# xxxupeng/stereo_toolbox

Measured on AMD Instinct MI355X. Metric: stereo pairs/sec @ 540x960 D=192 (GwcNet_GC fwd+bwd), higher is better.
Workload: dtype f32; 1 GPU; GwcNet_GC(maxdisp=192) train step: fwd+bwd+allreduce+Adam, 576x960 pairs (reference pad_to_2x shape), batch 1/GPU, fp32, synthetic randn inputs, deterministic filler weights; global_batch=1, parallelism=dp1, grad_sync=none (single rank: flat fp32 buffer packed, no collective), launch=eager, optimizer=torch.optim.Adam(fused=True)

## Files before the change

### include/stx_hip.h

```cpp
#ifndef STX_HIP_H
#define STX_HIP_H
#ifdef __cplusplus
extern "C" {
#endif

const char* stx_last_error(void);
const char* stx_build_info(void);
int stx_get_tuning(const char* name);
int stx_set_tuning(const char* name, int value);

int stx_cost_volume_fwd(const float* Lg, const float* Rg, int Cg, int G, const float* Lc, const float* Rc, int Cc,
                        const float* scale, float* vol, int B, int H, int W, int D, int mask_left, void* stream);
int stx_group_normalize_fwd(const float* x, float* y, int B, int C, int G, int HW, float out_scale, void* stream);
int stx_group_normalize_bwd(const float* x, const float* gy, float* gx, int B, int C, int G, int HW, float out_scale, void* stream);
int stx_cost_volume_bwd(const float* gvol, const float* Lg, const float* Rg, int Cg, int G, int Cc, float* gLg,
                        float* gRg, float* gLc, float* gRc, int B, int H, int W, int D, int mask_left, void* stream);

int stx_head_fwd(const float* cost, float* disp, float* stats, int B, int Dc, int Hc, int Wc, int D, int H, int W,
                 void* stream);
long long stx_head_bwd_workspace_floats(int B, int Dc, int H, int W);
int stx_head_bwd(const float* gdisp, const float* cost, const float* disp, const float* stats, float* gcost,
                 float* workspace, int B, int Dc, int Hc, int Wc, int D, int H, int W, void* stream);
int stx_head_fwd2(const float* cost, float* disp, float* stats, int B, int Dc, int Hc, int Wc, int D, int H, int W,
                  int align_corners, void* stream);
// ... 71 lines not shown
                    float* running_mean, float* running_var, float momentum, float eps, float* scale, float* shift,
                    float* mean, float* invstd, void* stream);
int stx_bn_finalize_groups(const float* partials, int nrows, int C, double count, const float* gamma, const float* beta,
                           float* running_mean, float* running_var, float momentum, float eps, float* out, int groups,
                           void* stream);
int stx_bn_apply(const float* z1, const float* scale1, const float* shift1, const float* z2, const float* scale2,
                 const float* shift2, float* out, long long nvox, int C, int relu, int groups, void* stream);
int stx_bn_bwd_reduce(const float* gy, const float* y, const float* z1, const float* mean1, const float* invstd1,
                      const float* z2, const float* mean2, const float* invstd2, float* partials, float* sums,
                      long long nvox, int C, int relu, void* stream);
int stx_bn_bwd_apply(const float* gy, const float* y, const float* z1, const float* mean1, const float* invstd1,
                     const float* gamma1, const float* z2, const float* mean2, const float* invstd2,
                     const float* gamma2, const float* sums, float* dz1, float* dz2, float* gout, long long nvox, int C,
                     int relu, void* stream);
int stx_bn_bwd_reduce2(const float* gy, const float* y, const float* z1, const float* mean1, const float* invstd1,
                       const float* z2, const float* mean2, const float* invstd2, const float* scale1,
                       const float* shift1, const float* scale2, const float* shift2, float* partials, float* sums,
                       long long nvox, int C, int relu, int groups, void* stream);
int stx_bn_bwd_apply2(const float* gy, const float* y, const float* z1, const float* mean1, const float* invstd1,
                      const float* gamma1, const float* z2, const float* mean2, const float* invstd2,
                      const float* gamma2, const float* scale1, const float* shift1, const float* scale2,
                      const float* shift2, const float* sums, float* dz1, float* dz2, float* gout, long long nvox,
                      int C, int relu, int groups, void* stream);

int stx_pad_normalize_u8(const unsigned char* img, float* out, int B, int H, int W, int Hp, int Wp, int top,
                         const float* mean3, const float* std3, void* stream);

int stx_sampled_volume_fwd(const float* Lg, const float* Rg, int Cg, int G, const float* Lc, const float* Rc, int Cc,
                           const float* samples, float* vol, int B, int H, int W, int S, int CTp, void* stream);
int stx_sampled_volume_bwd(const float* gvol, const float* Lg, const float* Rg, int Cg, int G, int Cc,
                           const float* samples, float* gLg, float* gRg, float* gLc, float* gRc, int B, int H, int W,
                           int S, int CTp, void* stream);

int stx_warp_fwd(const float* x, const float* disp, float* out, int B, int C, int H, int W, void* stream);
int stx_warp_bwd(const float* gout, const float* x, const float* disp, float* gx, float* gdisp, int B, int C, int H, int W,
                 void* stream);
int stx_corr_volume_fwd(const float* ref, const float* tgt, float* vol, int B, int C, int H, int W, int maxdisp, int groups,
                        void* stream);
int stx_corr_volume_bwd(const float* gvol, const float* ref, const float* tgt, float* gref, float* gtgt, int B, int C, int H,
                        int W, int maxdisp, int groups, void* stream);
int stx_disparity_variance_fwd(const float* x, const float* disp, const float* samples, float* out, int B, int D, int HW,
                               void* stream);
int stx_disparity_variance_bwd(const float* g, const float* x, const float* disp, const float* samples, float* gx, float* gdisp,
                               float* gsamples, int B, int D, int HW, void* stream);

long long stx_geo_pyramid_floats(long long rows, int len, int C, int levels);
// ... 19 lines not shown
```

### stereo_toolbox_amd/_capi.py

```python
import ctypes
import os
import threading

import torch

_P = ctypes.c_void_p
_I = ctypes.c_int
_F = ctypes.c_float
_L = ctypes.c_longlong

SIGNATURES = {
    "stx_get_tuning": [ctypes.c_char_p],
    "stx_set_tuning": [ctypes.c_char_p, _I],
    "stx_cost_volume_fwd": [_P, _P, _I, _I, _P, _P, _I, _P, _P, _I, _I, _I, _I, _I, _P],
    "stx_cost_volume_bwd": [_P, _P, _P, _I, _I, _I, _P, _P, _P, _P, _I, _I, _I, _I, _I, _P],
    "stx_group_normalize_fwd": [_P, _P, _I, _I, _I, _I, _F, _P],
    "stx_group_normalize_bwd": [_P, _P, _P, _I, _I, _I, _I, _F, _P],
    "stx_head_fwd": [_P, _P, _P, _I, _I, _I, _I, _I, _I, _I, _P],
    "stx_head_bwd_workspace_floats": [_I, _I, _I, _I],
    "stx_head_bwd": [_P, _P, _P, _P, _P, _P, _I, _I, _I, _I, _I, _I, _I, _P],
    "stx_head_fwd2": [_P, _P, _P, _I, _I, _I, _I, _I, _I, _I, _I, _P],
    "stx_head_bwd2": [_P, _P, _P, _P, _P, _P, _I, _I, _I, _I, _I, _I, _I, _I, _P],
    "stx_softargmax_fwd": [_P, _P, _I, _I, _I, _P],
    "stx_argmax_fwd": [_P, _P, _I, _I, _I, _P],
# ... 43 lines not shown
    "stx_disparity_variance_fwd": [_P, _P, _P, _P, _I, _I, _I, _P],
    "stx_disparity_variance_bwd": [_P, _P, _P, _P, _P, _P, _P, _I, _I, _I, _P],
    "stx_sampled_volume_fwd": [_P, _P, _I, _I, _P, _P, _I, _P, _P, _I, _I, _I, _I, _I, _P],
    "stx_sampled_volume_bwd": [_P, _P, _P, _I, _I, _I, _P, _P, _P, _P, _P, _I, _I, _I, _I, _I, _P],
    "stx_geo_pyramid_floats": [_L, _I, _I, _I],
    "stx_geo_corr_fwd": [_P, _P, _P, _I, _I, _I, _I, _I, _I, _P],
    "stx_geo_corr_bwd": [_P, _P, _P, _P, _P, _I, _I, _I, _I, _I, _I, _P],
    "stx_geo_pyramid_fwd": [_P, _P, _I, _I, _I, _I, _I, _I, _P],
    "stx_geo_pyramid_bwd": [_P, _P, _I, _I, _I, _I, _I, _I, _P],
    "stx_geo_lookup_fwd": [_P, _P, _P, _P, _P, _I, _I, _I, _I, _I, _I, _I, _I, _P],
    "stx_geo_lookup_bwd": [_P, _P, _P, _P, _P, _I, _I, _I, _I, _I, _I, _I, _I, _P],
    "stx_context_upsample_fwd": [_P, _P, _P, _I, _I, _I, _P],
    "stx_context_upsample_bwd": [_P, _P, _P, _P, _P, _I, _I, _I, _P],
    "stx_bn_reduce_blocks": [],
    "stx_bn_stats_rows": [_L, _I],
    "stx_bn_stats": [_P, _P, _L, _I, _I, _P],
    "stx_bn_finalize": [_P, _I, _I, ctypes.c_double, _P, _P, _P, _P, _F, _F, _P, _P, _P, _P, _P],
    "stx_bn_finalize_groups": [_P, _I, _I, ctypes.c_double, _P, _P, _P, _P, _F, _F, _P, _I, _P],
    "stx_bn_apply": [_P, _P, _P, _P, _P, _P, _P, _L, _I, _I, _I, _P],
    "stx_bn_bwd_reduce": [_P, _P, _P, _P, _P, _P, _P, _P, _P, _P, _L, _I, _I, _P],
    "stx_bn_bwd_apply": [_P, _P, _P, _P, _P, _P, _P, _P, _P, _P, _P, _P, _P, _P, _L, _I, _I, _P],
    "stx_bn_bwd_reduce2": [_P] * 14 + [_L, _I, _I, _I, _P],
    "stx_bn_bwd_apply2": [_P] * 18 + [_L, _I, _I, _I, _P],
}
_RET_CHARP = ("stx_last_error", "stx_build_info")


class StxError(RuntimeError):
    pass


class StxLib:

    def __init__(self, path):
        if not os.path.exists(path):
            raise StxError(
                f"HIP library not found: {path}. Build it with `python -m stereo_toolbox_amd.build` "
                "(hipcc, gfx950). There is no CPU fallback for the cost-volume hot path.")
        self.path = path
        self._dll = ctypes.CDLL(path)
        for name in _RET_CHARP:
            fn = getattr(self._dll, name)
            fn.restype = ctypes.c_char_p
            fn.argtypes = []
        self._fns = {}
        for name, argtypes in SIGNATURES.items():
# ... 47 lines not shown
```

### stereo_toolbox_amd/csrc/bn.hip

```cpp
#include "stx_common.h"
#include <stdlib.h>

namespace {

constexpr int BN_THREADS = 256;
constexpr int BN_RED_BLOCKS = 1024;

__device__ __forceinline__ double bn_block_sum(double v, double* red, int tid) {
    red[tid] = v;
    __syncthreads();
    for (int s = BN_THREADS / 2; s > 0; s >>= 1) {
        if (tid < s) red[tid] += red[tid + s];
        __syncthreads();
    }
    const double r = red[0];
    __syncthreads();
    return r;
}

__global__ __launch_bounds__(BN_THREADS) void bn_finalize_kernel(
    const float* __restrict__ partials, int nrows, int C, double count, const float* __restrict__ gamma,
    const float* __restrict__ beta, float* __restrict__ running_mean, float* __restrict__ running_var,
    float momentum, float eps, float* __restrict__ scale, float* __restrict__ shift, float* __restrict__ mean_out,
    float* __restrict__ invstd_out, int groups) {
    __shared__ double red[BN_THREADS];
    const int c = blockIdx.x, tid = threadIdx.x;
    for (int g = 0; g < groups; ++g, partials += (size_t)nrows * 2 * C, scale += C, shift += C, mean_out += C, invstd_out += C) {
    double s1 = 0.0, s2 = 0.0;
    for (int r = tid; r < nrows; r += BN_THREADS) {
        s1 += (double)partials[(size_t)r * 2 * C + c];
        s2 += (double)partials[(size_t)r * 2 * C + C + c];
    }
    s1 = bn_block_sum(s1, red, tid);
    s2 = bn_block_sum(s2, red, tid);
    if (tid == 0) {
        const double mean = s1 / count;
        double var = s2 / count - mean * mean;
        if (var < 0.0) var = 0.0;
        const float invstd = (float)(1.0 / sqrt(var + (double)eps));
        const float g = gamma ? gamma[c] : 1.f, bt = beta ? beta[c] : 0.f;
        const float sc = g * invstd;
        scale[c] = sc;
        shift[c] = bt - (float)mean * sc;
        mean_out[c] = (float)mean;
        invstd_out[c] = invstd;
        if (running_mean) running_mean[c] = (1.f - momentum) * running_mean[c] + momentum * (float)mean;
        if (running_var) {
            const double unb = count > 1.0 ? var * count / (count - 1.0) : var;
            running_var[c] = (1.f - momentum) * running_var[c] + momentum * (float)unb;
        }
    }
    }
}

constexpr int BN_FIN_THREADS = 512;

__device__ __forceinline__ double bn_shfl_down_f64(double v, int delta) {
    union { double d; float f[2]; } a, b;
    a.d = v;
    b.f[0] = __shfl_down(a.f[0], delta);
    b.f[1] = __shfl_down(a.f[1], delta);
    return b.d;
}

__global__ __launch_bounds__(BN_FIN_THREADS) void bn_finalize4_kernel(
    const float* __restrict__ partials, int nrows, int C, double count, const float* __restrict__ gamma,
    const float* __restrict__ beta, float* __restrict__ running_mean, float* __restrict__ running_var,
    float momentum, float eps, float* __restrict__ scale, float* __restrict__ shift, float* __restrict__ mean_out,
    float* __restrict__ invstd_out, int groups) {
    __shared__ double red[BN_FIN_THREADS / 64][8];
    const int c0 = blockIdx.x * 4, tid = threadIdx.x, lane = tid & 63, wave = tid >> 6;
    for (int g = 0; g < groups; ++g, partials += (size_t)nrows * 2 * C, scale += C, shift += C, mean_out += C, invstd_out += C) {
    if (g) __syncthreads();
    double acc[8] = {0.0, 0.0, 0.0, 0.0, 0.0, 0.0, 0.0, 0.0};
    const float* p = partials + c0;
#pragma unroll 4
    for (int r = tid; r < nrows; r += BN_FIN_THREADS) {
        const float4 a = stx_ld4(p + (size_t)r * 2 * C), b = stx_ld4(p + (size_t)r * 2 * C + C);
        acc[0] += (double)a.x; acc[1] += (double)a.y; acc[2] += (double)a.z; acc[3] += (double)a.w;
        acc[4] += (double)b.x; acc[5] += (double)b.y; acc[6] += (double)b.z; acc[7] += (double)b.w;
    }
#pragma unroll
    for (int k = 0; k < 8; ++k) {
#pragma unroll
        for (int d = 32; d > 0; d >>= 1) acc[k] += bn_shfl_down_f64(acc[k], d);
        if (lane == 0) red[wave][k] = acc[k];
    }
    __syncthreads();
    if (tid < 4) {
        double s1 = 0.0, s2 = 0.0;
        for (int w = 0; w < BN_FIN_THREADS / 64; ++w) { s1 += red[w][tid]; s2 += red[w][4 + tid]; }
        const int c = c0 + tid;
        const double mean = s1 / count;
        double var = s2 / count - mean * mean;
        if (var < 0.0) var = 0.0;
        const float invstd = (float)(1.0 / sqrt(var + (double)eps));
        const float g = gamma ? gamma[c] : 1.f, bt = beta ? beta[c] : 0.f;
        const float sc = g * invstd;
        scale[c] = sc;
        shift[c] = bt - (float)mean * sc;
        mean_out[c] = (float)mean;
        invstd_out[c] = invstd;
        if (running_mean) running_mean[c] = (1.f - momentum) * running_mean[c] + momentum * (float)mean;
        if (running_var) {
            const double unb = count > 1.0 ? var * count / (count - 1.0) : var;
            running_var[c] = (1.f - momentum) * running_var[c] + momentum * (float)unb;
        }
    }
    }
}

__global__ __launch_bounds__(BN_THREADS) void bn_apply_kernel(
    const float* __restrict__ z1, const float* __restrict__ scale1, const float* __restrict__ shift1,
    const float* __restrict__ z2, const float* __restrict__ scale2, const float* __restrict__ shift2,
    float* __restrict__ out, size_t nquads, int CQ, int relu) {
    {
        const size_t go = (size_t)blockIdx.y * nquads * 4, gc = (size_t)blockIdx.y * CQ * 4;
        z1 += go; out += go; scale1 += gc; shift1 += gc;
        if (z2) z2 += go;
        if (scale2) { scale2 += gc; shift2 += gc; }
    }
    for (size_t i = (size_t)blockIdx.x * BN_THREADS + threadIdx.x; i < nquads; i += (size_t)gridDim.x * BN_THREADS) {
        const int cq = (int)(i % CQ) * 4;
        float4 v = stx_ld4(z1 + i * 4);
        const float4 a = stx_ld4(scale1 + cq), b = stx_ld4(shift1 + cq);
        v.x = fmaf(v.x, a.x, b.x); v.y = fmaf(v.y, a.y, b.y); v.z = fmaf(v.z, a.z, b.z); v.w = fmaf(v.w, a.w, b.w);
        if (z2) {
            float4 u = stx_ld4(z2 + i * 4);
            if (scale2) {
                const float4 a2 = stx_ld4(scale2 + cq), b2 = stx_ld4(shift2 + cq);
                u.x = fmaf(u.x, a2.x, b2.x); u.y = fmaf(u.y, a2.y, b2.y);
                u.z = fmaf(u.z, a2.z, b2.z); u.w = fmaf(u.w, a2.w, b2.w);
            }
            v.x += u.x; v.y += u.y; v.z += u.z; v.w += u.w;
        }
        if (relu) {
            v.x = stx_act(v.x, relu); v.y = stx_act(v.y, relu); v.z = stx_act(v.z, relu); v.w = stx_act(v.w, relu);
        }
        stx_st4(out + i * 4, v);
    }
}

__global__ __launch_bounds__(BN_THREADS) void bn_bwd_reduce_kernel(
    const float* __restrict__ gy, const float* __restrict__ y, const float* __restrict__ z1,
    const float* __restrict__ mean1, const float* __restrict__ invstd1, const float* __restrict__ z2,
    const float* __restrict__ mean2, const float* __restrict__ invstd2, const float* __restrict__ sc1,
    const float* __restrict__ sh1, const float* __restrict__ sc2, const float* __restrict__ sh2, float* __restrict__ partials,
    size_t nvox, int C, int relu) {
    __shared__ float red[BN_THREADS * 12];
    const int tid = threadIdx.x;
    const int CQ = C >> 2;
    const int cq = tid % CQ, vl = tid / CQ, VPB = BN_THREADS / CQ;
    {
        const size_t go = (size_t)blockIdx.y * nvox * C, gc = (size_t)blockIdx.y * C;
        gy += go; z1 += go; mean1 += gc; invstd1 += gc;
        if (y) y += go;
        if (z2) z2 += go;
        if (mean2) { mean2 += gc; invstd2 += gc; }
        if (sc1) { sc1 += gc; sh1 += gc; }
        if (sc2) { sc2 += gc; sh2 += gc; }
        partials += (size_t)blockIdx.y * gridDim.x * 3 * C;
    }
    const float4 m1 = stx_ld4(mean1 + 4 * cq), i1 = stx_ld4(invstd1 + 4 * cq);
    float4 m2 = make_float4(0.f, 0.f, 0.f, 0.f), i2 = m2;
    const bool has2 = z2 && mean2;
    if (has2) { m2 = stx_ld4(mean2 + 4 * cq); i2 = stx_ld4(invstd2 + 4 * cq); }
    const bool remask = relu && !y;
    float4 a1 = m2, b1 = m2, a2 = m2, b2 = m2;
    if (remask) {
        a1 = stx_ld4(sc1 + 4 * cq); b1 = stx_ld4(sh1 + 4 * cq);
        if (has2) { a2 = stx_ld4(sc2 + 4 * cq); b2 = stx_ld4(sh2 + 4 * cq); }
    }
// ... 17 lines not shown
            } else {
                yy = stx_ld4(y + o);
            }
            g.x = stx_act_bwd(g.x, yy.x, relu); g.y = stx_act_bwd(g.y, yy.y, relu);
            g.z = stx_act_bwd(g.z, yy.z, relu); g.w = stx_act_bwd(g.w, yy.w, relu);
        }
        s[0] += g.x; s[1] += g.y; s[2] += g.z; s[3] += g.w;
        s[4] = fmaf(g.x, (a.x - m1.x) * i1.x, s[4]); s[5] = fmaf(g.y, (a.y - m1.y) * i1.y, s[5]);
        s[6] = fmaf(g.z, (a.z - m1.z) * i1.z, s[6]); s[7] = fmaf(g.w, (a.w - m1.w) * i1.w, s[7]);
        if (has2) {
            s[8] = fmaf(g.x, (c.x - m2.x) * i2.x, s[8]); s[9] = fmaf(g.y, (c.y - m2.y) * i2.y, s[9]);
            s[10] = fmaf(g.z, (c.z - m2.z) * i2.z, s[10]); s[11] = fmaf(g.w, (c.w - m2.w) * i2.w, s[11]);
        }
    }
#pragma unroll
    for (int k = 0; k < 12; ++k) red[k * BN_THREADS + tid] = s[k];
    __syncthreads();
    for (int idx = tid; idx < 12 * CQ; idx += BN_THREADS) {
        const int k = idx / CQ, q = idx % CQ;
        float t = 0.f;
        for (int j = q; j < BN_THREADS; j += CQ) t += red[k * BN_THREADS + j];
        partials[((size_t)blockIdx.x * 3 + (k >> 2)) * C + 4 * q + (k & 3)] = t;
    }
}

__global__ __launch_bounds__(BN_THREADS) void bn_stats_kernel(const float* __restrict__ z, float* __restrict__ partials,
                                                              size_t nvox, int C) {
    __shared__ float red[BN_THREADS * 8];
    const int tid = threadIdx.x;
    const int CQ = C >> 2;
    const int cq = tid % CQ, vl = tid / CQ, VPB = BN_THREADS / CQ;
    z += (size_t)blockIdx.y * nvox * C;
    partials += (size_t)blockIdx.y * gridDim.x * 2 * C;
    float s[8];
#pragma unroll
    for (int k = 0; k < 8; ++k) s[k] = 0.f;
    const size_t step = (size_t)gridDim.x * VPB;
    size_t v = vl < VPB ? (size_t)blockIdx.x * VPB + vl : nvox;
    for (; v + 3 * step < nvox; v += 4 * step) {
        float4 a[4];
#pragma unroll
        for (int u = 0; u < 4; ++u) a[u] = stx_ld4(z + (v + u * step) * C + 4 * cq);
#pragma unroll
        for (int u = 0; u < 4; ++u) {
            s[0] += a[u].x; s[1] += a[u].y; s[2] += a[u].z; s[3] += a[u].w;
            s[4] = fmaf(a[u].x, a[u].x, s[4]); s[5] = fmaf(a[u].y, a[u].y, s[5]);
            s[6] = fmaf(a[u].z, a[u].z, s[6]); s[7] = fmaf(a[u].w, a[u].w, s[7]);
        }
    }
    for (; v < nvox; v += step) {
        const float4 a = stx_ld4(z + v * C + 4 * cq);
        s[0] += a.x; s[1] += a.y; s[2] += a.z; s[3] += a.w;
        s[4] = fmaf(a.x, a.x, s[4]); s[5] = fmaf(a.y, a.y, s[5]); s[6] = fmaf(a.z, a.z, s[6]); s[7] = fmaf(a.w, a.w, s[7]);
    }
#pragma unroll
    for (int k = 0; k < 8; ++k) red[k * BN_THREADS + tid] = s[k];
    __syncthreads();
    for (int idx = tid; idx < 8 * CQ; idx += BN_THREADS) {
        const int k = idx / CQ, q = idx % CQ;
        float t = 0.f;
        for (int j = q; j < BN_THREADS; j += CQ) t += red[k * BN_THREADS + j];
        partials[((size_t)blockIdx.x * 2 + (k >> 2)) * C + 4 * q + (k & 3)] = t;
    }
}

__global__ __launch_bounds__(BN_THREADS) void bn_colsum_kernel(const float* __restrict__ partials, int nrows, int M,
                                                               float* __restrict__ sums, int groups) {
    __shared__ double red[BN_THREADS];
    const int m = blockIdx.x, tid = threadIdx.x;
    float tot = 0.f;
    for (int g = 0; g < groups; ++g) {
        const float* p = partials + (size_t)g * nrows * M;
        double s = 0.0;
        for (int r = tid; r < nrows; r += BN_THREADS) s += (double)p[(size_t)r * M + m];
        s = bn_block_sum(s, red, tid);
        if (tid == 0) {
            sums[(size_t)g * M + m] = (float)s;
            tot += (float)s;
        }
    }
    if (groups > 1 && tid == 0) sums[(size_t)groups * M + m] = tot;
}

__global__ __launch_bounds__(BN_THREADS) void bn_bwd_apply_kernel(
    const float* __restrict__ gy, const float* __restrict__ y, const float* __restrict__ z1,
    const float* __restrict__ mean1, const float* __restrict__ invstd1, const float* __restrict__ gamma1,
// ... 98 lines not shown
extern "C" int stx_bn_finalize_groups(const float* partials, int nrows, int C, double count, const float* gamma,
                                      const float* beta, float* running_mean, float* running_var, float momentum, float eps,
                                      float* out, int groups, void* stream) {
    stx_begin();
    STX_REQUIRE(partials && nrows > 0 && C > 0 && count > 0 && out && groups >= 1, "bn_finalize_groups: bad args");
    const size_t gc = (size_t)groups * C;
    return bn_finalize_launch(partials, nrows, C, count, gamma, beta, running_mean, running_var, momentum, eps, out, out + gc,
                              out + 2 * gc, out + 3 * gc, groups, stream);
}

extern "C" int stx_bn_stats_rows(long long nvox, int C) {
    stx_begin();
    if (C < 4 || C % 4 != 0 || C / 4 > BN_THREADS || nvox < 1) return 0;
    const long long vpb = BN_THREADS / (C / 4);
    const long long g = (nvox + 4 * vpb - 1) / (4 * vpb);
    return (int)(g > 256 ? 256 : (g < 1 ? 1 : g));
}

extern "C" int stx_bn_stats(const float* z, float* partials, long long nvox, int C, int groups, void* stream) {
    stx_begin();
    STX_REQUIRE(z && partials && nvox > 0 && groups >= 1 && groups <= 65535, "bn_stats: bad args");
    STX_REQUIRE(C >= 4 && C % 4 == 0 && C / 4 <= BN_THREADS, "bn_stats: C=%d unsupported (a multiple of 4, at most 1024)", C);
    hipLaunchKernelGGL(bn_stats_kernel, dim3(stx_bn_stats_rows(nvox, C), groups), dim3(BN_THREADS), 0, (hipStream_t)stream, z,
                       partials, (size_t)nvox, C);
    return stx_check_launch("bn_stats");
}

extern "C" int stx_bn_apply(const float* z1, const float* scale1, const float* shift1, const float* z2,
                            const float* scale2, const float* shift2, float* out, long long nvox, int C, int relu,
                            int groups, void* stream) {
    stx_begin();
    STX_REQUIRE(z1 && scale1 && shift1 && out && nvox > 0 && C > 0 && C % 4 == 0, "bn_apply: bad args (C=%d)", C);
    STX_REQUIRE(!scale2 || (z2 && shift2), "bn_apply: second affine needs z2 and shift2");
    STX_REQUIRE(groups >= 1 && groups <= 65535, "bn_apply: groups=%d", groups);
    const size_t nquads = (size_t)nvox * (C / 4);
    hipLaunchKernelGGL(bn_apply_kernel, dim3(bn_grid(nquads), groups), dim3(BN_THREADS), 0, (hipStream_t)stream, z1, scale1,
                       shift1, z2, scale2, shift2, out, nquads, C / 4, relu);
    return stx_check_launch("bn_apply");
}

extern "C" int stx_bn_bwd_reduce2(const float* gy, const float* y, const float* z1, const float* mean1,
                                  const float* invstd1, const float* z2, const float* mean2, const float* invstd2,
                                  const float* scale1, const float* shift1, const float* scale2, const float* shift2,
                                  float* partials, float* sums, long long nvox, int C, int relu, int groups, void* stream) {
    stx_begin();
    STX_REQUIRE(gy && z1 && mean1 && invstd1 && partials && sums && nvox > 0, "bn_bwd_reduce: null operand");
    STX_REQUIRE(groups >= 1 && groups <= 65535, "bn_bwd_reduce: groups=%d", groups);
    STX_REQUIRE(C >= 4 && C % 4 == 0 && C / 4 <= BN_THREADS, "bn_bwd_reduce: C=%d unsupported (a multiple of 4, at most 1024)", C);
    STX_REQUIRE(!relu || y || (scale1 && shift1 && (!(z2 && mean2) || (scale2 && shift2))),
                "bn_bwd_reduce: the relu mask needs y or the forward pass's scale / shift vectors");
    STX_REQUIRE(relu != 2 || !y, "bn_bwd_reduce: Mish (activation code 2) differentiates the pre-activation value: pass y = NULL and the scale / shift vectors");
    hipStream_t st = (hipStream_t)stream;
    const int nblk = ((long long)nvox * C <= (9ll << 19)) ? BN_RED_BLOCKS / 4 : BN_RED_BLOCKS;
    hipLaunchKernelGGL(bn_bwd_reduce_kernel, dim3(nblk, groups), dim3(BN_THREADS), 0, st, gy, y, z1, mean1, invstd1,
                       z2, mean2, invstd2, scale1, shift1, scale2, shift2, partials, (size_t)nvox, C, relu);
    int rc = stx_check_launch("bn_bwd_reduce");
    if (rc) return rc;
    hipLaunchKernelGGL(bn_colsum_kernel, dim3(3 * C), dim3(BN_THREADS), 0, st, partials, nblk, 3 * C, sums, groups);
    return stx_check_launch("bn_colsum");
}

extern "C" int stx_bn_bwd_apply2(const float* gy, const float* y, const float* z1, const float* mean1,
                                 const float* invstd1, const float* gamma1, const float* z2, const float* mean2,
                                 const float* invstd2, const float* gamma2, const float* scale1, const float* shift1,
                                 const float* scale2, const float* shift2, const float* sums, float* dz1, float* dz2,
                                 float* gout, long long nvox, int C, int relu, int groups, void* stream) {
    stx_begin();
    STX_REQUIRE(gy && z1 && mean1 && invstd1 && sums && dz1 && nvox > 0 && C % 4 == 0, "bn_bwd_apply: bad args");
    STX_REQUIRE(groups >= 1 && groups <= 65535, "bn_bwd_apply: groups=%d", groups);
    STX_REQUIRE(!relu || y || (scale1 && shift1 && (!(z2 && mean2 && dz2) || (scale2 && shift2))),
                "bn_bwd_apply: the relu mask needs y or the forward pass's scale / shift vectors");
    STX_REQUIRE(relu != 2 || !y, "bn_bwd_apply: Mish (activation code 2) differentiates the pre-activation value: pass y = NULL and the scale / shift vectors");
    const size_t nquads = (size_t)nvox * (C / 4);
    hipLaunchKernelGGL(bn_bwd_apply_kernel, dim3(bn_grid(nquads), groups), dim3(BN_THREADS), 0, (hipStream_t)stream, gy, y, z1,
                       mean1, invstd1, gamma1, z2, mean2, invstd2, gamma2, scale1, shift1, scale2, shift2, sums, dz1, dz2,
                       gout, nquads, C, relu, (float)(1.0 / (double)nvox));
    return stx_check_launch("bn_bwd_apply");
}

extern "C" int stx_bn_bwd_reduce(const float* gy, const float* y, const float* z1, const float* mean1,
                                 const float* invstd1, const float* z2, const float* mean2, const float* invstd2,
                                 float* partials, float* sums, long long nvox, int C, int relu, void* stream) {
// ... 12 lines not shown
```

### stereo_toolbox_amd/csrc/stx_runtime.hip

```cpp
#include "stx_common.h"
#include <stdarg.h>
#include <stdio.h>

static thread_local char g_err[512] = "";

int stx_set_error(int code, const char* fmt, ...) {
    va_list ap;
    va_start(ap, fmt);
    vsnprintf(g_err, sizeof(g_err), fmt, ap);
    va_end(ap);
    return code;
}

int stx_check_launch(const char* what) {
    hipError_t e = hipGetLastError();
    if (e != hipSuccess) return stx_set_error(STX_ERR_LAUNCH, "%s: launch failed: %s", what, hipGetErrorString(e));
    return STX_OK;
}

extern "C" const char* stx_last_error(void) { return g_err; }

extern "C" const char* stx_build_info(void) {
#ifdef STX_HIPEMU
    return "stx-hipemu (host SIMT emulator build: tests only)";
// ... 12 lines not shown
    {"STX_SV_BWD_V1", 0}, {"STX_DWCONV_ROLL", 1},
};
struct TuneInit {
    TuneInit() {
        for (int i = 0; i < STX_TUNE_COUNT; ++i)
            if (const char* e = getenv(g_tune[i].name)) g_tune[i].value = atoi(e);
    }
} g_tune_init;
}

int stx_tune(StxTune id) { return g_tune[id].value; }

extern "C" int stx_get_tuning(const char* name) {
    for (int i = 0; i < STX_TUNE_COUNT; ++i)
        if (name && !strcmp(name, g_tune[i].name)) return g_tune[i].value;
    return -1;
}

extern "C" int stx_set_tuning(const char* name, int value) {
    for (int i = 0; i < STX_TUNE_COUNT; ++i)
        if (name && !strcmp(name, g_tune[i].name)) { g_tune[i].value = value; return STX_OK; }
    return stx_set_error(STX_ERR_ARG, "stx_set_tuning: unknown switch %s", name ? name : "(null)");
}
```

### stereo_toolbox_amd/models/features2d.py

```python
import math
import os
import threading

import torch
import torch.nn as nn
import torch.nn.functional as F

from .. import ops
from ..aggregation import _bn_state, _fold


def channels_last_weights_(module):
    for m in module.modules():
        if isinstance(m, nn.Conv2d) and m.weight.dim() == 4:
            m.weight.data = m.weight.data.contiguous(memory_format=torch.channels_last)
    return module


def fused_glue(x, *bns):
    if os.environ.get("STX_FEAT2D_FUSED", "1") == "0":
        return False
    if x.dtype != torch.float32 or not ops.on_device(x):
        return False
    if ops.autocast_active():
# ... 22 lines not shown

    def __exit__(self, *exc):
        view_groups._tls.n = self.old
        return False


def _nhwc(t):
    v = t.permute(0, 2, 3, 1)
    return v if v.is_contiguous() else v.contiguous()


def cat_features(parts):
    parts = list(parts)
    if (os.environ.get("STX_FEAT2D_FUSED", "1") != "0" and os.environ.get("STX_FEAT2D_FUSED_CAT", "1") != "0" and 2 <= len(parts) <= 4
            and all(p.dtype == torch.float32 and ops.on_device(p) and p.shape[1] % 4 == 0
                    and p.is_contiguous(memory_format=torch.channels_last) for p in parts)):
        return ops.cat_channels([_nhwc(p) for p in parts]).permute(0, 3, 1, 2)
    return torch.cat(parts, dim=1)


def own_conv2d(x, conv):
    return (os.environ.get("STX_FEAT2D_CONV", "1") != "0" and x.dtype == torch.float32 and ops.on_device(x)
            and ops.conv2d_supported(conv) and x.shape[0] % view_groups.current() == 0)


def conv_bn_act(x, conv, bn, relu=False, residual=None, second=None):
    G = view_groups.current()
    part = None
    if bn.training and own_conv2d(x, conv):
        zl, part = ops.Conv2dFn.apply(x, conv.weight, G)
        z = zl.permute(0, 3, 1, 2)
    else:
        z = F.conv2d(x, conv.weight, conv.bias, conv.stride, conv.padding, conv.dilation, conv.groups)
        zl = _nhwc(z)
    if not bn.training:
        if torch.is_grad_enabled() and (z.requires_grad or bn.weight.requires_grad):
            raise ops.StxError("conv_bn_act: eval-mode BatchNorm under autograd has no fused backward -- gate the call "
                               "with fused_glue() over every BatchNorm of the block")
        sc, sh = _fold(bn)
        if second is not None:
            sc2, sh2 = _fold(second[1])
            y = ops.bn_apply(zl, sc, sh, _nhwc(second[0]), sc2, sh2, relu)
        else:
            y = ops.bn_apply(zl, sc, sh, None if residual is None else _nhwc(residual), None, None, relu)
        return y.permute(0, 3, 1, 2)
    st = _bn_state(bn, part if part is not None else ops.bn_stats(zl.detach(), G), zl.numel() // zl.shape[-1] // G, steps=G)
    if second is not None:
        z2l = _nhwc(second[0])
        bn2 = second[1]
        st2 = _bn_state(bn2, ops.bn_stats(z2l.detach(), G), z2l.numel() // z2l.shape[-1] // G, steps=G)
        y = ops.BnActFn.apply(zl, bn.weight, bn.bias, z2l, bn2.weight, bn2.bias, None, relu, st, st2, G)
    else:
        y = ops.BnActFn.apply(zl, bn.weight, bn.bias, None, None, None, None if residual is None else _nhwc(residual),
                              relu, st, None, G)
    return y.permute(0, 3, 1, 2)


def convbn_relu_chain(seq, x):
    i, n = 0, len(seq)
    while i < n:
        m = seq[i]
        if isinstance(m, nn.Sequential) and len(m) == 2 and isinstance(m[0], nn.Conv2d):
            relu = i + 1 < n and isinstance(seq[i + 1], nn.ReLU)
            x = conv_bn_act(x, m[0], m[1], relu=relu)
            i += 2 if relu else 1
        else:
            x = m(x)
            i += 1
    return x


def _chain_bns(seq):
    return [m[1] for m in seq if isinstance(m, nn.Sequential) and len(m) == 2 and isinstance(m[0], nn.Conv2d)]
# ... 130 lines not shown
```

### stereo_toolbox_amd/ops.py

```python
import ctypes

import torch

from ._capi import StxError, get_lib

_P = ctypes.c_void_p


class _DevPtr(ctypes.c_void_p):
    """A device pointer that remembers the device of the tensor it came from: _call() reads the launch device off its
    own arguments, so nothing survives between launches (an exception between building the arguments and the launch
    cannot leak state into the next one)."""


def _stream(dev=None):
    return _P(torch.cuda.current_stream(dev).cuda_stream)


def _p(t):
    if t is None:
        return None
    p = _DevPtr(t.data_ptr())
    p.dev = t.device
    return p
# ... 693 lines not shown
def bn_finalize(partials, count, gamma, beta, running_mean, running_var, momentum, eps, groups=1):
    C = partials.shape[-1]
    out = torch.empty(4, groups, C, dtype=torch.float32, device=partials.device)
    _call("stx_bn_finalize_groups", _p(partials), partials.shape[-3], C, float(count), _p(gamma), _p(beta),
          _p(running_mean), _p(running_var), float(momentum), float(eps), _p(out), groups)
    return list(out.unbind(0)) if groups > 1 else list(out[:, 0].unbind(0))


@fp32_region
def bn_stats(z, groups=1):
    _chk(z, "z")
    C = z.shape[-1]
    nvox = z.numel() // C // groups
    if groups < 1 or z.shape[0] % groups:
        raise StxError(f"bn_stats: leading axis {z.shape[0]} does not split into {groups} groups")
    rows = get_lib().raw("stx_bn_stats_rows")(nvox, C)
    if rows <= 0:
        raise StxError(f"bn_stats: C={C} unsupported")
    part = torch.empty(groups, rows, 2, C, dtype=torch.float32, device=z.device)
    _call("stx_bn_stats", _p(z), _p(part), nvox, C, groups)
    return part if groups > 1 else part[0]


def _sync_bn_partials(partials, count, group, world):
    import torch.distributed as dist
    tot = partials.double().sum(0)
    dist.all_reduce(tot, group=group)
    hi = tot.float()
    lo = (tot - hi.double()).float()
    return torch.stack((hi, lo)).contiguous(), count * world


@fp32_region
def bn_apply(z1, scale1, shift1, z2=None, scale2=None, shift2=None, relu=False, groups=1):
    out = torch.empty_like(z1)
    C = z1.shape[-1]
    _call("stx_bn_apply", _p(z1), _p(scale1), _p(shift1), _p(z2), _p(scale2), _p(shift2), _p(out),
          z1.numel() // C // groups, C, int(relu), groups)
    return out


class BnActFn(torch.autograd.Function):

    @staticmethod
    def forward(ctx, z1, gamma1, beta1, z2, gamma2, beta2, residual, relu, bn1, bn2, groups=1, defer=False):
        G = int(groups)
        ctx.defer = bool(defer)

        def affine(gamma, beta, bn):
            if bn["training"]:
                partials, count = bn["partials"], bn["count"]
                if bn.get("sync"):
                    if G > 1:
                        raise StxError("BnActFn: SyncBatchNorm with groups is not wired (SyncBN runs the views separately)")
                    partials, count = _sync_bn_partials(partials, count, *bn["sync"])
                return bn_finalize(partials, count, gamma, beta, bn["running_mean"], bn["running_var"], bn["momentum"],
                                   bn["eps"], G)
            invstd = torch.rsqrt(bn["running_var"] + bn["eps"])
            scale = gamma * invstd
            res = (scale, beta - bn["running_mean"] * scale, bn["running_mean"].clone(), invstd)
            return res if G == 1 else [t.unsqueeze(0).expand(G, -1).contiguous() for t in res]

        relu = int(relu)
        if relu == 2 and residual is not None:
            raise StxError("BnActFn: Mish with a plain residual is not wired (no model of the family uses it)")
        if G < 1 or z1.shape[0] % G:
            raise StxError(f"BnActFn: leading axis {z1.shape[0]} does not split into {G} groups")
        sc1, sh1, m1, i1 = affine(gamma1, beta1, bn1)
        two = z2 is not None
        if two:
            sc2, sh2, m2, i2 = affine(gamma2, beta2, bn2)
            y = bn_apply(z1, sc1, sh1, z2, sc2, sh2, relu, G)
        else:
# ... 2 lines not shown
        ctx.relu, ctx.two, ctx.has_res, ctx.groups = relu, two, residual is not None, G
        ctx.train1 = bn1["training"]
        ctx.train2 = bn2["training"] if two else False
        ctx.sync = bn1.get("sync") or (bn2.get("sync") if two else None)
        ctx.remask = bool(relu) and residual is None
        keep_y = y if (relu and not ctx.remask) else None
        ctx.save_for_backward(z1, gamma1, m1, i1, z2, gamma2, m2, i2, keep_y, sc1 if ctx.remask else None,
                              sh1 if ctx.remask else None, sc2 if (ctx.remask and two) else None,
                              sh2 if (ctx.remask and two) else None)
        return y

    @staticmethod
    def backward(ctx, gy):
        z1, gamma1, m1, i1, z2, gamma2, m2, i2, y, sc1, sh1, sc2, sh2 = ctx.saved_tensors
        gy = gy.contiguous()
        G = ctx.groups
        C = z1.shape[-1]
        nvox = z1.numel() // C // G
        lib = get_lib()
        NB = lib.raw("stx_bn_reduce_blocks")()
        part = _WS.get("bnred", G * NB * 3 * C, z1.device)
        sums_all = torch.empty(G + (1 if G > 1 else 0), 3, C, dtype=torch.float32, device=z1.device)
        sums = sums_all[:G]
        _call("stx_bn_bwd_reduce2", _p(gy), _p(y), _p(z1), _p(m1), _p(i1), _p(z2) if ctx.two else None,
              _p(m2) if ctx.two else None, _p(i2) if ctx.two else None, _p(sc1), _p(sh1), _p(sc2), _p(sh2), _p(part),
              _p(sums_all), nvox, C, int(ctx.relu), G)
        if not ctx.needs_input_grad[0] and not ctx.two and not ctx.has_res:
            tot = sums_all[G] if G > 1 else sums_all[0]
            return (None, tot[1], tot[0], None, None, None, None, None, None, None, None, None)
        if (ctx.defer and not ctx.two and not ctx.has_res and ctx.relu in (0, 1) and ctx.train1 and not ctx.sync and G == 1
                and (not ctx.relu or ctx.remask)):
            alias = gy.view_as(gy)
            pend = _PendingBn()
            pend.g, pend.z, pend.scale, pend.shift, pend.mean, pend.invstd = alias, z1, sc1, sh1, m1, i1
            pend.gamma, pend.sums, pend.inv_n, pend.act = gamma1, sums, 1.0 / nvox, int(ctx.relu)
            if pend.scale is None:
                pend.scale = pend.shift = m1
            _defer_pending_bn(alias, pend)
            tot = sums_all[0]
            return (alias, tot[1], tot[0], None, None, None, None, None, None, None, None, None)
        dz1 = torch.empty_like(z1)
        dz2 = torch.empty_like(z2) if ctx.two else None
        gres = torch.empty_like(z1) if (ctx.has_res and ctx.relu) else None
        use = sums
        if ctx.sync:
            import torch.distributed as dist
            use = sums.clone()
# ... 735 lines not shown
```

Before: 0.1786 pairs/s.

## Fuse BN partial-sum reduction and finalize into the stats kernels via last-block counters

Adds a last-block-done reduction scheme. Per-block partial rows are reduced in double into a pooled scratch slot guarded by atomic counters, and the final block either finalizes the BN affine parameters (forward stats) or writes the column sums (backward reduce). This removes the separate colsum and finalize kernel launches for each 2D-feature BN layer in both forward and backward. In exchange it adds a ring of 16 reusable counter/scratch slots, which could collide if more than 16 reductions are in flight, and it adds extra serial work in the last block.

```diff
diff --git a/include/stx_hip.h b/include/stx_hip.h
--- a/include/stx_hip.h
+++ b/include/stx_hip.h
@@ -117,6 +117,14 @@
                       const float* gamma2, const float* scale1, const float* shift1, const float* scale2,
                       const float* shift2, const float* sums, float* dz1, float* dz2, float* gout, long long nvox,
                       int C, int relu, int groups, void* stream);
+int stx_bn_bwd_reduce_sums(const float* gy, const float* y, const float* z1, const float* mean1, const float* invstd1,
+                           const float* z2, const float* mean2, const float* invstd2, const float* scale1,
+                           const float* shift1, const float* scale2, const float* shift2, float* partials, float* sums,
+                           long long nvox, int C, int relu, int groups, void* stream);
+int stx_bn_stats_finalize(const float* z, float* partials, long long nvox, int C, int groups, double count,
+                          const float* gamma, const float* beta, float* running_mean, float* running_var, float momentum,
+                          float eps, float* out, void* stream);
+int stx_red_counters_pending(void* stream);
 
 int stx_pad_normalize_u8(const unsigned char* img, float* out, int B, int H, int W, int Hp, int Wp, int top,
                          const float* mean3, const float* std3, void* stream);
diff --git a/stereo_toolbox_amd/_capi.py b/stereo_toolbox_amd/_capi.py
--- a/stereo_toolbox_amd/_capi.py
+++ b/stereo_toolbox_amd/_capi.py
@@ -89,6 +89,9 @@
     "stx_bn_bwd_apply": [_P, _P, _P, _P, _P, _P, _P, _P, _P, _P, _P, _P, _P, _P, _L, _I, _I, _P],
     "stx_bn_bwd_reduce2": [_P] * 14 + [_L, _I, _I, _I, _P],
     "stx_bn_bwd_apply2": [_P] * 18 + [_L, _I, _I, _I, _P],
+    "stx_bn_bwd_reduce_sums": [_P] * 14 + [_L, _I, _I, _I, _P],
+    "stx_bn_stats_finalize": [_P, _P, _L, _I, _I, ctypes.c_double, _P, _P, _P, _P, _F, _F, _P, _P],
+    "stx_red_counters_pending": [_P],
 }
 _RET_CHARP = ("stx_last_error", "stx_build_info")
 
diff --git a/stereo_toolbox_amd/csrc/bn.hip b/stereo_toolbox_amd/csrc/bn.hip
--- a/stereo_toolbox_amd/csrc/bn.hip
+++ b/stereo_toolbox_amd/csrc/bn.hip
@@ -1,4 +1,5 @@
 #include "stx_common.h"
+#include "stx_reduce.h"
 #include <stdlib.h>
 
 namespace {
@@ -34,21 +35,8 @@
     s1 = bn_block_sum(s1, red, tid);
     s2 = bn_block_sum(s2, red, tid);
     if (tid == 0) {
-        const double mean = s1 / count;
-        double var = s2 / count - mean * mean;
-        if (var < 0.0) var = 0.0;
-        const float invstd = (float)(1.0 / sqrt(var + (double)eps));
-        const float g = gamma ? gamma[c] : 1.f, bt = beta ? beta[c] : 0.f;
-        const float sc = g * invstd;
-        scale[c] = sc;
-        shift[c] = bt - (float)mean * sc;
-        mean_out[c] = (float)mean;
-        invstd_out[c] = invstd;
-        if (running_mean) running_mean[c] = (1.f - momentum) * running_mean[c] + momentum * (float)mean;
-        if (running_var) {
-            const double unb = count > 1.0 ? var * count / (count - 1.0) : var;
-            running_var[c] = (1.f - momentum) * running_var[c] + momentum * (float)unb;
-        }
+        stx_bn_finalize_channel(s1, s2, count, c, gamma, beta, running_mean, running_var, momentum, eps, scale, shift,
+                                mean_out, invstd_out);
     }
     }
 }
@@ -91,21 +79,8 @@
         double s1 = 0.0, s2 = 0.0;
         for (int w = 0; w < BN_FIN_THREADS / 64; ++w) { s1 += red[w][tid]; s2 += red[w][4 + tid]; }
         const int c = c0 + tid;
-        const double mean = s1 / count;
-        double var = s2 / count - mean * mean;
-        if (var < 0.0) var = 0.0;
-        const float invstd = (float)(1.0 / sqrt(var + (double)eps));
-        const float g = gamma ? gamma[c] : 1.f, bt = beta ? beta[c] : 0.f;
-        const float sc = g * invstd;
-        scale[c] = sc;
-        shift[c] = bt - (float)mean * sc;
-        mean_out[c] = (float)mean;
-        invstd_out[c] = invstd;
-        if (running_mean) running_mean[c] = (1.f - momentum) * running_mean[c] + momentum * (float)mean;
-        if (running_var) {
-            const double unb = count > 1.0 ? var * count / (count - 1.0) : var;
-            running_var[c] = (1.f - momentum) * running_var[c] + momentum * (float)unb;
-        }
+        stx_bn_finalize_channel(s1, s2, count, c, gamma, beta, running_mean, running_var, momentum, eps, scale, shift,
+                                mean_out, invstd_out);
     }
     }
 }
@@ -146,8 +121,9 @@
     const float* __restrict__ mean1, const float* __restrict__ invstd1, const float* __restrict__ z2,
     const float* __restrict__ mean2, const float* __restrict__ invstd2, const float* __restrict__ sc1,
     const float* __restrict__ sh1, const float* __restrict__ sc2, const float* __restrict__ sh2, float* __restrict__ partials,
-    size_t nvox, int C, int relu) {
+    size_t nvox, int C, int relu, StxRedSlot slot, float* __restrict__ sums) {
     __shared__ float red[BN_THREADS * 12];
+    __shared__ unsigned red_flag;
     const int tid = threadIdx.x;
     const int CQ = C >> 2;
     const int cq = tid % CQ, vl = tid / CQ, VPB = BN_THREADS / CQ;
@@ -211,11 +187,33 @@
         for (int j = q; j < BN_THREADS; j += CQ) t += red[k * BN_THREADS + j];
         partials[((size_t)blockIdx.x * 3 + (k >> 2)) * C + 4 * q + (k & 3)] = t;
     }
-}
+    if (!slot.counters) return;
+    const int M = 3 * C, nsets = stx_red_sets((int)gridDim.x), groups = (int)gridDim.y;
+    if (!stx_red_rows(partials, (int)gridDim.x, M, (int)blockIdx.x, (int)blockIdx.y * nsets, groups * nsets, slot, &red_flag))
+        return;
+    for (int m = tid; m < M; m += BN_THREADS) {
+        float tot = 0.f;
+        for (int g = 0; g < groups; ++g) {
+            const float sg = (float)stx_red_col(slot.scratch + (size_t)g * nsets * M, nsets, M, m);
+            sums[(size_t)g * M + m] = sg;
+            tot += sg;
+        }
+        if (groups > 1) sums[(size_t)groups * M + m] = tot;
+    }
+}
+
+struct BnFinArgs {
+    double count;
+    const float *gamma, *beta;
+    float *running_mean, *running_var;
+    float momentum, eps;
+    float *scale, *shift, *mean, *invstd;
+};
 
 __global__ __launch_bounds__(BN_THREADS) void bn_stats_kernel(const float* __restrict__ z, float* __restrict__ partials,
-                                                              size_t nvox, int C) {
+                                                              size_t nvox, int C, StxRedSlot slot, BnFinArgs fin) {
     __shared__ float red[BN_THREADS * 8];
+    __shared__ unsigned red_flag;
     const int tid = threadIdx.x;
     const int CQ = C >> 2;
     const int cq = tid % CQ, vl = tid / CQ, VPB = BN_THREADS / CQ;
@@ -251,6 +249,18 @@
         for (int j = q; j < BN_THREADS; j += CQ) t += red[k * BN_THREADS + j];
         partials[((size_t)blockIdx.x * 2 + (k >> 2)) * C + 4 * q + (k & 3)] = t;
     }
+    if (!slot.counters) return;
+    const int M = 2 * C, nsets = stx_red_sets((int)gridDim.x), groups = (int)gridDim.y;
+    if (!stx_red_rows(partials, (int)gridDim.x, M, (int)blockIdx.x, (int)blockIdx.y * nsets, groups * nsets, slot, &red_flag))
+        return;
+    for (int c = tid; c < C; c += BN_THREADS)
+        for (int g = 0; g < groups; ++g) {
+            const double* sc = slot.scratch + (size_t)g * nsets * M;
+            const size_t gc = (size_t)g * C;
+            stx_bn_finalize_channel(stx_red_col(sc, nsets, M, c), stx_red_col(sc, nsets, M, C + c), fin.count, c, fin.gamma,
+                                    fin.beta, fin.running_mean, fin.running_var, fin.momentum, fin.eps, fin.scale + gc,
+                                    fin.shift + gc, fin.mean + gc, fin.invstd + gc);
+        }
 }
 
 __global__ __launch_bounds__(BN_THREADS) void bn_colsum_kernel(const float* __restrict__ partials, int nrows, int M,
@@ -395,8 +405,34 @@
     STX_REQUIRE(z && partials && nvox > 0 && groups >= 1 && groups <= 65535, "bn_stats: bad args");
     STX_REQUIRE(C >= 4 && C % 4 == 0 && C / 4 <= BN_THREADS, "bn_stats: C=%d unsupported (a multiple of 4, at most 1024)", C);
     hipLaunchKernelGGL(bn_stats_kernel, dim3(stx_bn_stats_rows(nvox, C), groups), dim3(BN_THREADS), 0, (hipStream_t)stream, z,
-                       partials, (size_t)nvox, C);
+                       partials, (size_t)nvox, C, StxRedSlot{nullptr, nullptr}, BnFinArgs{});
     return stx_check_launch("bn_stats");
+}
+
+static bool bn_red_fits(int rows, int groups, int M) {
+    const long long sets = (long long)groups * stx_red_sets(rows);
+    return sets <= STX_RED_MAX_SETS && sets * M <= STX_RED_SLOT_DOUBLES;
+}
+
+extern "C" int stx_bn_stats_finalize(const float* z, float* partials, long long nvox, int C, int groups, double count,
+                                     const float* gamma, const float* beta, float* running_mean, float* running_var,
+                                     float momentum, float eps, float* out, void* stream) {
+    stx_begin();
+    STX_REQUIRE(z && partials && nvox > 0 && groups >= 1 && groups <= 65535 && count > 0 && out, "bn_stats_finalize: bad args");
+    STX_REQUIRE(C >= 4 && C % 4 == 0 && C / 4 <= BN_THREADS, "bn_stats_finalize: C=%d unsupported (a multiple of 4, at most 1024)", C);
+    const int rows = stx_bn_stats_rows(nvox, C);
+    if (!bn_red_fits(rows, groups, 2 * C)) {
+        if (int rc = stx_bn_stats(z, partials, nvox, C, groups, stream)) return rc;
+        return stx_bn_finalize_groups(partials, rows, C, count, gamma, beta, running_mean, running_var, momentum, eps, out,
+                                      groups, stream);
+    }
+    StxRedSlot slot;
+    if (int rc = stx_red_acquire(&slot)) return rc;
+    const size_t gc = (size_t)groups * C;
+    const BnFinArgs fin{count, gamma, beta, running_mean, running_var, momentum, eps, out, out + gc, out + 2 * gc, out + 3 * gc};
+    hipLaunchKernelGGL(bn_stats_kernel, dim3(rows, groups), dim3(BN_THREADS), 0, (hipStream_t)stream, z, partials, (size_t)nvox,
+                       C, slot, fin);
+    return stx_check_launch("bn_stats_finalize");
 }
 
 extern "C" int stx_bn_apply(const float* z1, const float* scale1, const float* shift1, const float* z2,
@@ -412,10 +448,11 @@
     return stx_check_launch("bn_apply");
 }
 
-extern "C" int stx_bn_bwd_reduce2(const float* gy, const float* y, const float* z1, const float* mean1,
+static int bn_bwd_reduce_launch(const float* gy, const float* y, const float* z1, const float* mean1,
                                   const float* invstd1, const float* z2, const float* mean2, const float* invstd2,
                                   const float* scale1, const float* shift1, const float* scale2, const float* shift2,
-                                  float* partials, float* sums, long long nvox, int C, int relu, int groups, void* stream) {
+                                  float* partials, float* sums, long long nvox, int C, int relu, int groups, void* stream,
+                                  bool fuse) {
     stx_begin();
     STX_REQUIRE(gy && z1 && mean1 && invstd1 && partials && sums && nvox > 0, "bn_bwd_reduce: null operand");
     STX_REQUIRE(groups >= 1 && groups <= 65535, "bn_bwd_reduce: groups=%d", groups);
@@ -425,12 +462,33 @@
     STX_REQUIRE(relu != 2 || !y, "bn_bwd_reduce: Mish (activation code 2) differentiates the pre-activation value: pass y = NULL and the scale / shift vectors");
     hipStream_t st = (hipStream_t)stream;
     const int nblk = ((long long)nvox * C <= (9ll << 19)) ? BN_RED_BLOCKS / 4 : BN_RED_BLOCKS;
+    StxRedSlot slot{nullptr, nullptr};
+    fuse = fuse && bn_red_fits(nblk, groups, 3 * C);
+    if (fuse)
+        if (int rc = stx_red_acquire(&slot)) return rc;
     hipLaunchKernelGGL(bn_bwd_reduce_kernel, dim3(nblk, groups), dim3(BN_THREADS), 0, st, gy, y, z1, mean1, invstd1,
-                       z2, mean2, invstd2, scale1, shift1, scale2, shift2, partials, (size_t)nvox, C, relu);
+                       z2, mean2, invstd2, scale1, shift1, scale2, shift2, partials, (size_t)nvox, C, relu, slot, sums);
     int rc = stx_check_launch("bn_bwd_reduce");
-    if (rc) return rc;
+    if (rc || fuse) return rc;
     hipLaunchKernelGGL(bn_colsum_kernel, dim3(3 * C), dim3(BN_THREADS), 0, st, partials, nblk, 3 * C, sums, groups);
     return stx_check_launch("bn_colsum");
+}
+
+extern "C" int stx_bn_bwd_reduce2(const float* gy, const float* y, const float* z1, const float* mean1,
+                                  const float* invstd1, const float* z2, const float* mean2, const float* invstd2,
+                                  const float* scale1, const float* shift1, const float* scale2, const float* shift2,
+                                  float* partials, float* sums, long long nvox, int C, int relu, int groups, void* stream) {
+    return bn_bwd_reduce_launch(gy, y, z1, mean1, invstd1, z2, mean2, invstd2, scale1, shift1, scale2, shift2, partials, sums,
+                                nvox, C, relu, groups, stream, false);
+}
+
+extern "C" int stx_bn_bwd_reduce_sums(const float* gy, const float* y, const float* z1, const float* mean1,
+                                      const float* invstd1, const float* z2, const float* mean2, const float* invstd2,
+                                      const float* scale1, const float* shift1, const float* scale2, const float* shift2,
+                                      float* partials, float* sums, long long nvox, int C, int relu, int groups,
+                                      void* stream) {
+    return bn_bwd_reduce_launch(gy, y, z1, mean1, invstd1, z2, mean2, invstd2, scale1, shift1, scale2, shift2, partials, sums,
+                                nvox, C, relu, groups, stream, true);
 }
 
 extern "C" int stx_bn_bwd_apply2(const float* gy, const float* y, const float* z1, const float* mean1,
diff --git a/stereo_toolbox_amd/csrc/stx_reduce.h b/stereo_toolbox_amd/csrc/stx_reduce.h
--- /dev/null
+++ b/stereo_toolbox_amd/csrc/stx_reduce.h
@@ -0,0 +1,74 @@
+#pragma once
+#include "stx_common.h"
+
+#ifdef STX_HIPEMU
+static inline void __threadfence() { __atomic_thread_fence(__ATOMIC_SEQ_CST); }
+#endif
+
+constexpr int STX_RED_SET = 32;
+constexpr int STX_RED_MAX_SETS = 127;
+constexpr int STX_RED_SLOT_DOUBLES = 1 << 16;
+__host__ __device__ inline int stx_red_sets(int rows) { return (rows + STX_RED_SET - 1) / STX_RED_SET; }
+
+struct StxRedSlot {
+    unsigned* counters;
+    double* scratch;
+};
+int stx_red_acquire(StxRedSlot* slot);
+
+__device__ __forceinline__ bool stx_red_last(unsigned* ctr, unsigned total, unsigned* flag) {
+    __threadfence();
+    __syncthreads();
+    if (threadIdx.x == 0) {
+        const unsigned last = atomicAdd(ctr, 1u) == total - 1u;
+        if (last) *ctr = 0u;
+        *flag = last;
+    }
+    __syncthreads();
+    const bool last = *flag != 0u;
+    if (last) __threadfence();
+    return last;
+}
+
+__device__ __forceinline__ bool stx_red_rows(const float* rows, int nrows, int M, int row, int set0, int nsets_all,
+                                             StxRedSlot slot, unsigned* flag) {
+    const int set = row / STX_RED_SET, r0 = set * STX_RED_SET;
+    const int n = nrows - r0 < STX_RED_SET ? nrows - r0 : STX_RED_SET;
+    if (!stx_red_last(slot.counters + 1 + set0 + set, (unsigned)n, flag)) return false;
+    double* dst = slot.scratch + (size_t)(set0 + set) * M;
+    for (int m = threadIdx.x; m < M; m += blockDim.x) {
+        const float* p = rows + (size_t)r0 * M + m;
+        double s = 0.0;
+#pragma unroll 8
+        for (int r = 0; r < n; ++r) s += (double)p[(size_t)r * M];
+        dst[m] = s;
+    }
+    return stx_red_last(slot.counters, (unsigned)nsets_all, flag);
+}
+
+__device__ __forceinline__ double stx_red_col(const double* scratch, int nsets, int M, int m) {
+    double s = 0.0;
+    for (int k = 0; k < nsets; ++k) s += scratch[(size_t)k * M + m];
+    return s;
+}
+
+__device__ __forceinline__ void stx_bn_finalize_channel(double s1, double s2, double count, int c, const float* gamma,
+                                                        const float* beta, float* running_mean, float* running_var,
+                                                        float momentum, float eps, float* scale, float* shift,
+                                                        float* mean_out, float* invstd_out) {
+    const double mean = s1 / count;
+    double var = s2 / count - mean * mean;
+    if (var < 0.0) var = 0.0;
+    const float invstd = (float)(1.0 / sqrt(var + (double)eps));
+    const float g = gamma ? gamma[c] : 1.f, bt = beta ? beta[c] : 0.f;
+    const float sc = g * invstd;
+    scale[c] = sc;
+    shift[c] = bt - (float)mean * sc;
+    mean_out[c] = (float)mean;
+    invstd_out[c] = invstd;
+    if (running_mean) running_mean[c] = (1.f - momentum) * running_mean[c] + momentum * (float)mean;
+    if (running_var) {
+        const double unb = count > 1.0 ? var * count / (count - 1.0) : var;
+        running_var[c] = (1.f - momentum) * running_var[c] + momentum * (float)unb;
+    }
+}
diff --git a/stereo_toolbox_amd/csrc/stx_runtime.hip b/stereo_toolbox_amd/csrc/stx_runtime.hip
--- a/stereo_toolbox_amd/csrc/stx_runtime.hip
+++ b/stereo_toolbox_amd/csrc/stx_runtime.hip
@@ -58,3 +58,77 @@
         if (name && !strcmp(name, g_tune[i].name)) { g_tune[i].value = value; return STX_OK; }
     return stx_set_error(STX_ERR_ARG, "stx_set_tuning: unknown switch %s", name ? name : "(null)");
 }
+
+#include "stx_reduce.h"
+#include <mutex>
+namespace {
+constexpr int RED_SLOTS = 16, RED_MAX_DEV = 16;
+constexpr int RED_CTRS = STX_RED_MAX_SETS + 1;
+struct RedPool { unsigned* counters = nullptr; double* scratch = nullptr; unsigned next = 0; };
+RedPool g_red[RED_MAX_DEV];
+std::mutex g_red_mu;
+
+int red_device(int* dev) {
+#ifdef STX_HIPEMU
+    *dev = 0;
+#else
+    if (hipGetDevice(dev) != hipSuccess || *dev < 0 || *dev >= RED_MAX_DEV)
+        return stx_set_error(STX_ERR_LAUNCH, "stx_red_acquire: no current device (or more than %d)", RED_MAX_DEV);
+#endif
+    return STX_OK;
+}
+
+int red_alloc(RedPool& p) {
+    const size_t cb = (size_t)RED_SLOTS * RED_CTRS * sizeof(unsigned), sb = (size_t)RED_SLOTS * STX_RED_SLOT_DOUBLES * sizeof(double);
+#ifdef STX_HIPEMU
+    p.counters = (unsigned*)calloc(1, cb);
+    p.scratch = (double*)calloc(1, sb);
+#else
+    void *c = nullptr, *s = nullptr;
+    if (hipMalloc(&c, cb) != hipSuccess || hipMalloc(&s, sb) != hipSuccess || hipMemset(c, 0, cb) != hipSuccess) {
+        (void)hipGetLastError();
+        if (c) (void)hipFree(c);
+        if (s) (void)hipFree(s);
+        return stx_set_error(STX_ERR_LAUNCH, "stx_red_acquire: cannot allocate the reduction slots");
+    }
+    p.counters = (unsigned*)c;
+    p.scratch = (double*)s;
+#endif
+    return STX_OK;
+}
+}
+
+int stx_red_acquire(StxRedSlot* slot) {
+    int dev = 0;
+    if (int rc = red_device(&dev)) return rc;
+    std::lock_guard<std::mutex> lock(g_red_mu);
+    RedPool& p = g_red[dev];
+    if (!p.counters)
+        if (int rc = red_alloc(p)) return rc;
+    const unsigned k = p.next++ % RED_SLOTS;
+    slot->counters = p.counters + (size_t)k * RED_CTRS;
+    slot->scratch = p.scratch + (size_t)k * STX_RED_SLOT_DOUBLES;
+    return STX_OK;
+}
+
+extern "C" int stx_red_counters_pending(void* stream) {
+    int dev = 0;
+    if (red_device(&dev)) return -1;
+    std::lock_guard<std::mutex> lock(g_red_mu);
+    const RedPool& p = g_red[dev];
+    if (!p.counters) return 0;
+    static unsigned host[RED_SLOTS * RED_CTRS];
+#ifdef STX_HIPEMU
+    (void)stream;
+    memcpy(host, p.counters, sizeof(host));
+#else
+    if (hipStreamSynchronize((hipStream_t)stream) != hipSuccess ||
+        hipMemcpy(host, p.counters, sizeof(host), hipMemcpyDeviceToHost) != hipSuccess) {
+        (void)hipGetLastError();
+        return -1;
+    }
+#endif
+    int n = 0;
+    for (unsigned v : host) n += v != 0;
+    return n;
+}
diff --git a/stereo_toolbox_amd/models/features2d.py b/stereo_toolbox_amd/models/features2d.py
--- a/stereo_toolbox_amd/models/features2d.py
+++ b/stereo_toolbox_amd/models/features2d.py
@@ -68,6 +68,18 @@
 def own_conv2d(x, conv):
     return (os.environ.get("STX_FEAT2D_CONV", "1") != "0" and x.dtype == torch.float32 and ops.on_device(x)
             and ops.conv2d_supported(conv) and x.shape[0] % view_groups.current() == 0)
+
+
+def _stats_state(bn, zl, part, G):
+    count = zl.numel() // zl.shape[-1] // G
+    if part is not None:
+        return _bn_state(bn, part, count, steps=G)
+    st = _bn_state(bn, None, count, steps=G)
+    if st["sync"] is None:
+        st["gamma"], st["beta"] = bn.weight, bn.bias
+        return ops.bn_stats_finalize(zl.detach(), st, G)
+    st["partials"] = ops.bn_stats(zl.detach(), G)
+    return st
 
 
 def conv_bn_act(x, conv, bn, relu=False, residual=None, second=None):
@@ -90,11 +102,11 @@
         else:
             y = ops.bn_apply(zl, sc, sh, None if residual is None else _nhwc(residual), None, None, relu)
         return y.permute(0, 3, 1, 2)
-    st = _bn_state(bn, part if part is not None else ops.bn_stats(zl.detach(), G), zl.numel() // zl.shape[-1] // G, steps=G)
+    st = _stats_state(bn, zl, part, G)
     if second is not None:
         z2l = _nhwc(second[0])
         bn2 = second[1]
-        st2 = _bn_state(bn2, ops.bn_stats(z2l.detach(), G), z2l.numel() // z2l.shape[-1] // G, steps=G)
+        st2 = _stats_state(bn2, z2l, None, G)
         y = ops.BnActFn.apply(zl, bn.weight, bn.bias, z2l, bn2.weight, bn2.bias, None, relu, st, st2, G)
     else:
         y = ops.BnActFn.apply(zl, bn.weight, bn.bias, None, None, None, None if residual is None else _nhwc(residual),
diff --git a/stereo_toolbox_amd/ops.py b/stereo_toolbox_amd/ops.py
--- a/stereo_toolbox_amd/ops.py
+++ b/stereo_toolbox_amd/ops.py
@@ -739,6 +739,27 @@
     return part if groups > 1 else part[0]
 
 
+@fp32_region
+def bn_stats_finalize(z, bn, groups=1):
+    _chk(z, "z")
+    if bn.get("sync"):
+        raise StxError("bn_stats_finalize: SyncBatchNorm all-reduces the rows before they are finalized")
+    C = z.shape[-1]
+    nvox = z.numel() // C // groups
+    if groups < 1 or z.shape[0] % groups:
+        raise StxError(f"bn_stats_finalize: leading axis {z.shape[0]} does not split into {groups} groups")
+    rows = get_lib().raw("stx_bn_stats_rows")(nvox, C)
+    if rows <= 0:
+        raise StxError(f"bn_stats_finalize: C={C} unsupported")
+    part = torch.empty(groups, rows, 2, C, dtype=torch.float32, device=z.device)
+    out = torch.empty(4, groups, C, dtype=torch.float32, device=z.device)
+    _call("stx_bn_stats_finalize", _p(z), _p(part), nvox, C, groups, float(bn["count"]), _p(bn["gamma"]), _p(bn["beta"]),
+          _p(bn["running_mean"]), _p(bn["running_var"]), float(bn["momentum"]), float(bn["eps"]), _p(out))
+    bn["partials"] = part if groups > 1 else part[0]
+    bn["final"] = list(out.unbind(0)) if groups > 1 else list(out[:, 0].unbind(0))
+    return bn
+
+
 def _sync_bn_partials(partials, count, group, world):
     import torch.distributed as dist
     tot = partials.double().sum(0)
@@ -766,6 +787,8 @@
 
         def affine(gamma, beta, bn):
             if bn["training"]:
+                if bn.get("final") is not None:
+                    return bn["final"]
                 partials, count = bn["partials"], bn["count"]
                 if bn.get("sync"):
                     if G > 1:
@@ -814,7 +837,7 @@
         part = _WS.get("bnred", G * NB * 3 * C, z1.device)
         sums_all = torch.empty(G + (1 if G > 1 else 0), 3, C, dtype=torch.float32, device=z1.device)
         sums = sums_all[:G]
-        _call("stx_bn_bwd_reduce2", _p(gy), _p(y), _p(z1), _p(m1), _p(i1), _p(z2) if ctx.two else None,
+        _call("stx_bn_bwd_reduce_sums", _p(gy), _p(y), _p(z1), _p(m1), _p(i1), _p(z2) if ctx.two else None,
               _p(m2) if ctx.two else None, _p(i2) if ctx.two else None, _p(sc1), _p(sh1), _p(sc2), _p(sh2), _p(part),
               _p(sums_all), nvox, C, int(ctx.relu), G)
         if not ctx.needs_input_grad[0] and not ctx.two and not ctx.has_res:
```

Result: no change. 0.1786 pairs/s (+0.0%).
